# apple/ml-neuman

Hardware: AMD Instinct MI355X
Metric: rays_per_sec (800x800 frame, 128 samples/ray coarse + 128 importance, NeuMan background NeRF) (higher is better)
Workload: dtype coarse (sampling) pass: split-fp16 hi+lo MFMA x3, f32 accumulate; fine (shading) pass: per-row-scaled int16 as two int8 limbs on the i8 MFMA x3, exact int32 accumulate, encodings on split bf16

## Files before the change

ml-neuman_amd/csrc/mlp_host.hip:

```cpp
#include <stdarg.h>
#include <stdio.h>
#include <stdlib.h>
#include <string.h>

#include <vector>

#include "common.h"
#include "mlp_layout.h"
#include "mlp_launch.h"

namespace nm {

static thread_local char g_err[512] = "";

void set_error(const char* fmt, ...) {
    va_list ap;
    va_start(ap, fmt);
    vsnprintf(g_err, sizeof(g_err), fmt, ap);
    va_end(ap);
}
int check_hip(hipError_t e, const char* what) {
    if (e == hipSuccess) return NM_OK;
    set_error("%s: %s", what, hipGetErrorString(e));
    return NM_ERR_HIP;
// ... 302 lines not shown
                                int v = (int)lrintf(w / q[n]);
                                if (v > kFixedMax) v = kFixedMax;
                                if (v < -kFixedMax) v = -kFixedMax;
                                const int l = ((v + 128) & 255) - 128;
                                const int h = (v - l) >> 8;
                                hi[(g * 32 + r) * 16 + e] = (int8_t)h;
                                lo[(g * 32 + r) * 16 + e] = (int8_t)l;
                            }
                    }
                }
        }
        for (int n = 0; n < nrows; ++n) b[n] /= u[n];
        for (int nb = 0; nb < sh.nblk; ++nb)
            for (int t = 0; t < sh.bfsteps; ++t) {
                uint16_t* hi = reinterpret_cast<uint16_t*>(img + frag_off8(st, nb, sh.i8steps + t));
                uint16_t* lo = hi + 64 * 8;
                const int cc0 = st == 9 ? 32 : 0;
                for (int lane = 0; lane < 64; ++lane)
                    for (int j = 0; j < 8; ++j) {
                        const int n = 32 * nb + (lane & 31);
                        const float wv = stage_weight(d, P, st, n, cc0 + 2 * t + (lane >> 5), j) / u[n];
                        const uint16_t h = f32_to_bf16(wv);
                        hi[lane * 8 + j] = h;
                        lo[lane * 8 + j] = f32_to_bf16(wv - bf16_to_f32(h));
                    }
            }
    }
}

static void pack_stream8s(const uint8_t* img8, uint8_t* out, bool plain = false) {
    memset(out, 0, (size_t)(kWeightBytes8 + kWeightPadBytes));
    uint8_t* dst = out;
    auto put = [&](int st, int nb, int t0, int n) {
        for (int t = 0; t < n; ++t, dst += kStepBytes) memcpy(dst, img8 + frag_off8(st, nb, t0 + t), (size_t)kStepBytes);
    };
    for (int nb = 0; nb < 8; ++nb) put(0, nb, 0, 4);
    for (int st = 1; st <= 7; ++st) {
        for (int nb = 0; nb < 8; ++nb) put(st, nb, 0, 8);
        if (st == 5)
            for (int nb = 0; nb < 8; ++nb) put(5, nb, 8, 4);
    }
    put(8, 8, 0, 8);
    if (plain) {
        for (int nb = 0; nb < 2; ++nb) { put(0, nb, 0, 4); dst += 4 * kStepBytes; }
        if (dst - out != kPlainStreamBytes8) abort();
        return;
    }
    for (int nb = 0; nb < 8; ++nb) put(8, nb, 0, 8);
    for (int nb = 0; nb < 4; ++nb) put(9, nb, 0, 10);
    put(10, 0, 0, 4);
    if (dst - out != kWeightBytes8) abort();
}

constexpr int kSigmaSteps = 8 * 4 + 6 * 8 * 16 + 8 * 20 + 16;
static void sigma_stream_table(std::vector<int>& tab, int ndir) {
    tab.clear();
    std::vector<int> direct;
    auto put = [&](int st, int b, int t0, int n) {
        for (int t = 0; t < n; ++t)
            for (int k = 0; k < 4; ++k) {
                const int off = (int)frag_off(st, b + (k >> 1), t0 + t) + 1024 * (k & 1);
                (k < 4 - ndir ? tab : direct).push_back(off);
            }
    };
    for (int st = 0; st <= 7; ++st) {
        const StageShape sh = stage_shape(st);
        for (int b = 0; b < 8; b += 2) {
            if (sh.pe_steps) put(st, b, 0, sh.pe_steps);
            for (int t0 = sh.pe_steps; t0 < sh.steps; t0 += 8) put(st, b, t0, 8);
        }
    }
    for (int t = 0; t < 16; ++t) { tab.push_back((int)frag_off(8, 8, t)); tab.push_back((int)frag_off(8, 8, t) + 1024); }
    tab.insert(tab.end(), direct.begin(), direct.end());
    if ((int)tab.size() != 2 * kSigmaSteps) abort();
}
__global__ void sigma_stream_kernel(const uint4* __restrict__ image, const int* __restrict__ tab, int npieces, uint4* __restrict__ out) {
    const int i = blockIdx.x * blockDim.x + threadIdx.x;
    if (i >= npieces * 64) return;
    out[i] = image[tab[i >> 6] / 16 + (i & 63)];
}

static void pack_stream8(const uint8_t* img8, uint8_t* out) {
    memset(out, 0, (size_t)kWeightBytes8w);
    for (int q = 0; q < 4; ++q) {
        uint8_t* dst = out + wstream_off(q);
        auto put = [&](int st, int nb, int t0, int n) {
            for (int t = 0; t < n; ++t, dst += kStepBytes) memcpy(dst, img8 + frag_off8(st, nb, t0 + t), (size_t)kStepBytes);
        };
        put(0, 2 * q, 0, 4); put(0, 2 * q + 1, 0, 4);
        for (int st = 1; st <= 8; ++st) {
            put(st, 2 * q, 0, 8); put(st, 2 * q + 1, 0, 8);
            if (st == 5) { put(5, 2 * q, 8, 4); put(5, 2 * q + 1, 8, 4); }
        }
        if (q < 2) put(8, 8, 0, 8);
        put(9, q, 0, 8); put(9, q, 8, 2);
        dst += 2 * kStepBytes;
        if (q < 2) put(10, 0, 0, 4);
        dst += kW8Pad * kStepBytes;
        if (dst != out + wstream_off(q) + (int64_t)wstream_steps(q) * kStepBytes) abort();
    }
}

}

struct nm_mlp_s {
    nm_mlp_desc desc;
// ... 39 lines not shown
int nm_mlp_pack_f16(const nm_mlp_desc* desc, const float* const* host_params, void* host_out) {
    if (int e = nm::validate_desc(desc)) return e;
    NM_REQUIRE(host_params && host_out, "nm_mlp_pack_f16: null pointer");
    for (int i = 0; i < (desc->plain_head ? 18 : 24); ++i) NM_REQUIRE(host_params[i], "nm_mlp_pack_f16: host_params[%d] is null", i);
    nm::pack_image(desc, host_params, static_cast<uint8_t*>(host_out), true);
    return NM_OK;
}

int64_t nm_mlp_pack_i8_bytes(const nm_mlp_desc* desc) {
    if (nm::validate_desc(desc) != NM_OK) return -1;
    return nm::image8_bytes();
}

int nm_mlp_pack_i8(const nm_mlp_desc* desc, const float* const* host_params, void* host_out) {
    if (int e = nm::validate_desc(desc)) return e;
    NM_REQUIRE(host_params && host_out, "nm_mlp_pack_i8: null pointer");
    for (int i = 0; i < (desc->plain_head ? 18 : 24); ++i) NM_REQUIRE(host_params[i], "nm_mlp_pack_i8: host_params[%d] is null", i);
    nm::pack_image8(desc, host_params, static_cast<uint8_t*>(host_out));
    return NM_OK;
}

int64_t nm_mlp_pack_i8s_bytes(const nm_mlp_desc* desc) {
    if (nm::validate_desc(desc) != NM_OK) return -1;
    return nm::kWeightBytes8 + nm::kWeightPadBytes;
}

int nm_mlp_pack_i8s(const nm_mlp_desc* desc, const float* const* host_params, void* host_out) {
    if (int e = nm::validate_desc(desc)) return e;
    NM_REQUIRE(host_params && host_out, "nm_mlp_pack_i8s: null pointer");
    for (int i = 0; i < (desc->plain_head ? 18 : 24); ++i) NM_REQUIRE(host_params[i], "nm_mlp_pack_i8s: host_params[%d] is null", i);
    std::vector<uint8_t> img8((size_t)nm::image8_bytes());
    nm::pack_image8(desc, host_params, img8.data());
    nm::pack_stream8s(img8.data(), static_cast<uint8_t*>(host_out), desc->plain_head != 0);
    return NM_OK;
}

int nm_mlp_create(const nm_mlp_desc* desc, const float* const* host_params, const float* host_pos_tab,
                  const float* host_dir_tab, nm_mlp_t* out) {
    if (int e = nm::validate_desc(desc)) return e;
    NM_REQUIRE(host_params && host_pos_tab && host_dir_tab && out, "nm_mlp_create: null pointer");
    const int plain = desc->plain_head;
    for (int i = 0; i < (plain ? 18 : 24); ++i) NM_REQUIRE(host_params[i], "nm_mlp_create: host_params[%d] is null", i);
    const int64_t bytes = nm_mlp_pack_bytes(desc);
    std::vector<uint8_t> img((size_t)bytes);
    nm::pack_image(desc, host_params, img.data());
    std::vector<uint8_t> img16((size_t)bytes);
    nm::pack_image(desc, host_params, img16.data(), true);
    std::vector<uint8_t> img8((size_t)nm::image8_bytes());
    std::vector<uint8_t> str8((size_t)nm::kWeightBytes8w);
    std::vector<uint8_t> str8s((size_t)(nm::kWeightBytes8 + nm::kWeightPadBytes));
    nm::pack_image8(desc, host_params, img8.data());
    nm::pack_stream8(img8.data(), str8.data());
    nm::pack_stream8s(img8.data(), str8s.data(), plain != 0);

    const int kpe = 3 + 6 * desc->pos_n_freqs, kdpe = 3 + 6 * desc->dir_n_freqs;
    const int K[12] = {kpe, 256, 256, 256, 256, kpe + 256, 256, 256, plain ? 0 : 256 + kdpe, plain ? 0 : 256, 256, plain ? 0 : 128};
    const int N[12] = {256, 256, 256, 256, 256, 256, 256, 256, plain ? 0 : 128, plain ? 0 : 256, plain ? 4 : 1, plain ? 0 : 3};
    const int src[12] = {0, 2, 4, 6, 8, 10, 12, 14, 16, 18, plain ? (int)nm::P_OUT_W : 20, 22};
    nm_mlp_s* m = new nm_mlp_s();
    m->desc = *desc;
    int woff = 0;
    for (int l = 0; l < 12; ++l) { m->ref_off[l] = woff; woff += K[l] * N[l]; }
    int boff = woff;
    for (int l = 0; l < 12; ++l) { m->ref_boff[l] = boff; boff += N[l]; }
    std::vector<float> ref((size_t)boff);
    for (int l = 0; l < 12; ++l) {
        if (!K[l]) continue;
        const float* W = host_params[src[l]];
        for (int k = 0; k < K[l]; ++k)
            for (int n = 0; n < N[l]; ++n) ref[m->ref_off[l] + (size_t)k * N[l] + n] = W[(size_t)n * K[l] + k];
        memcpy(&ref[m->ref_boff[l]], host_params[src[l] + 1], (size_t)N[l] * 4);
    }
    float tab[192];
    memset(tab, 0, sizeof(tab));
    const int npos = desc->pe_kind == NM_PE_POSENC ? desc->pos_n_freqs : 9 * desc->pos_n_freqs;
    const int ndir = desc->pe_kind == NM_PE_POSENC ? desc->dir_n_freqs : 9 * desc->dir_n_freqs;
    memcpy(tab, host_pos_tab, (size_t)npos * 4);
    memcpy(tab + 96, host_dir_tab, (size_t)ndir * 4);
    auto octaves = [&](const float* t, int nfreq) {
        const int per = desc->pe_kind == NM_PE_POSENC ? 1 : 9;
        for (int b = 0; b + 1 < nfreq; ++b)
            for (int k = 0; k < per; ++k)
                if (t[(b + 1) * per + k] != 2.f * t[b * per + k]) return 0;
        return 1;
    };
    m->pos_octaves = octaves(tab, desc->pos_n_freqs);
    m->dir_octaves = octaves(tab + 96, desc->dir_n_freqs);

    m->d_image = nullptr; m->d_image16 = nullptr; m->d_consts8 = nullptr; m->d_stream8 = nullptr; m->d_image8 = nullptr; m->d_stream16t = nullptr; m->d_sigma_tab = nullptr; m->d_bwd_image = nullptr; m->d_petab = nullptr; m->d_ref = nullptr; m->d_wscale16 = nullptr;
    int rc = nm::check_hip(hipMalloc(&m->d_image, (size_t)bytes), "nm_mlp_create: hipMalloc(image)");
    const size_t consts_off = (size_t)(nm::kWeightBytes8 + nm::kWeightPadBytes), consts_bytes = img8.size() - consts_off;
    if (!rc) rc = nm::check_hip(hipMalloc(&m->d_consts8, consts_bytes), "nm_mlp_create: hipMalloc(consts8)");
    if (!rc) rc = nm::check_hip(hipMemcpy(m->d_consts8, img8.data() + consts_off, consts_bytes, hipMemcpyHostToDevice), "nm_mlp_create: upload consts8");
    if (!rc) rc = nm::check_hip(hipMalloc(&m->d_stream8, str8.size()), "nm_mlp_create: hipMalloc(stream8)");
    if (!rc) rc = nm::check_hip(hipMemcpy(m->d_stream8, str8.data(), str8.size(), hipMemcpyHostToDevice), "nm_mlp_create: upload stream8");
    if (!rc) rc = nm::check_hip(hipMalloc(&m->d_image8, consts_off), "nm_mlp_create: hipMalloc(image8)");
    if (!rc) rc = nm::check_hip(hipMemcpy(m->d_image8, str8s.data(), consts_off, hipMemcpyHostToDevice), "nm_mlp_create: upload image8");
    if (!rc) rc = nm::check_hip(hipMalloc(&m->d_petab, sizeof(tab)), "nm_mlp_create: hipMalloc(petab)");
    if (!rc) rc = nm::check_hip(hipMalloc(&m->d_ref, ref.size() * 4), "nm_mlp_create: hipMalloc(ref)");
    if (!rc) rc = nm::check_hip(hipMemcpy(m->d_image, img.data(), (size_t)bytes, hipMemcpyHostToDevice), "nm_mlp_create: upload image");
    if (!rc) rc = nm::check_hip(hipMalloc(&m->d_image16, (size_t)bytes), "nm_mlp_create: hipMalloc(image16)");
    if (!rc) rc = nm::check_hip(hipMemcpy(m->d_image16, img16.data(), (size_t)bytes, hipMemcpyHostToDevice), "nm_mlp_create: upload image16");
    if (!rc) rc = nm::check_hip(hipMemcpy(m->d_petab, tab, sizeof(tab), hipMemcpyHostToDevice), "nm_mlp_create: upload petab");
    if (!rc) rc = nm::check_hip(hipMemcpy(m->d_ref, ref.data(), ref.size() * 4, hipMemcpyHostToDevice), "nm_mlp_create: upload ref");
    if (!rc && !plain) {
        std::vector<int> stab;
// ... 42 lines not shown
}

int nm_mlp_destroy(nm_mlp_t m) {
    if (!m) return NM_OK;
    if (m->d_image) (void)hipFree(m->d_image);
    if (m->d_image16) (void)hipFree(m->d_image16);
    if (m->d_consts8) (void)hipFree(m->d_consts8);
    if (m->d_stream8) (void)hipFree(m->d_stream8);
    if (m->d_image8) (void)hipFree(m->d_image8);
    if (m->d_stream16t) (void)hipFree(m->d_stream16t);
    if (m->d_sigma_tab) (void)hipFree(m->d_sigma_tab);
    if (m->d_bwd_image) (void)hipFree(m->d_bwd_image);
    if (m->d_petab) (void)hipFree(m->d_petab);
    if (m->d_ref) (void)hipFree(m->d_ref);
    if (m->d_wscale16) (void)hipFree(m->d_wscale16);
    delete m;
    return NM_OK;
}

static int mlp_dispatch(nm_mlp_t m, const float* pts, const float* dirs, const float* origin, const float* direction,
                        const float* z, int64_t n, int S, int in_mode, int precision, int stop_stage, float sigma_scale,
                        float* out, float* dbg, nm_stream_t stream, void* prof = nullptr, int sigma_only = 0,
                        const nm::MlpChunk* chunk = nullptr) {
    NM_REQUIRE(m, "nm_mlp_forward: null handle");
    NM_REQUIRE(n >= 0, "nm_mlp_forward: negative n");
    NM_REQUIRE(precision == NM_PREC_FP32 || precision == NM_PREC_BF16X3 || precision == NM_PREC_BF16 || precision == NM_PREC_I8X3 ||
                   precision == NM_PREC_FP16X3,
               "nm_mlp_forward: bad precision %d", precision);
    if (n == 0) return NM_OK;
    NM_REQUIRE(!(chunk && precision == NM_PREC_FP32), "nm_mlp_forward_ray_chunk: the exact-f32 validation kernel has no chunked form");
    NM_REQUIRE(!(m->desc.plain_head && precision == NM_PREC_I8X3 && (stop_stage != -2 || dbg || prof || sigma_only)),
               "nm_mlp_forward: the plain-head (use_viewdirs=False) net's i8x3 form is the whole-network launch only (no stage-by-stage / density-only form)");
    NM_REQUIRE(!(m->desc.plain_head && stop_stage > 7), "nm_mlp_forward_debug: the plain-head net has stages -1..7 only");
    if (precision == NM_PREC_FP32) {
        nm::RefLaunch L;
        L.plain_head = m->desc.plain_head;
        L.wt = m->d_ref; L.bias = m->d_ref; L.petab = m->d_petab;
        for (int i = 0; i < 12; ++i) { L.off[i] = m->ref_off[i]; L.boff[i] = m->ref_boff[i]; }
        L.pe_kind = m->desc.pe_kind; L.pos_nfreq = m->desc.pos_n_freqs; L.dir_nfreq = m->desc.dir_n_freqs;
        return nm::launch_mlp_ref(L, pts, dirs, origin, direction, z, n, S, in_mode, stop_stage, sigma_scale, out, dbg,
                                  nm::as_stream(stream));
    }
    nm::MlpLaunch L;
    L.wpack = m->d_image;
    L.bias = reinterpret_cast<const float*>(m->d_image + nm::kWeightBytes + nm::kWeightPadBytes);
    L.wpack16 = m->d_image16;
    L.bias16 = reinterpret_cast<const float*>(m->d_image16 + nm::kWeightBytes + nm::kWeightPadBytes);
    L.petab = m->d_petab;
    L.pe_kind = m->desc.pe_kind; L.pos_nfreq = m->desc.pos_n_freqs; L.dir_nfreq = m->desc.dir_n_freqs;
    L.pos_octaves = m->pos_octaves; L.dir_octaves = m->dir_octaves;
    L.plain_head = m->desc.plain_head;
    L.wstream8 = m->d_stream8;
    L.consts8 = m->d_consts8;
    static const bool i8_as = [] { const char* e = getenv("NEUMAN_I8_KERNEL"); return !e || !strcmp(e, "as"); }();
    const char* sk = getenv("NEUMAN_SIGMA_KERNEL");
    const bool sigma_t = !(sk && !strcmp(sk, "w")) && m->d_stream16t;
    if (sigma_t && precision == NM_PREC_FP16X3 && sigma_only == 1 && stop_stage == -2 && !dbg && !prof && !m->desc.plain_head)
        return nm::launch_sigma_f16t(L, m->d_stream16t, m->sigma_ndir, pts, dirs, origin, direction, z, n, S, in_mode, sigma_scale, out, nm::as_stream(stream), chunk, nullptr, -1);
    if ((i8_as || m->desc.plain_head) && precision == NM_PREC_I8X3 && stop_stage == -2 && !dbg && !prof && !sigma_only)
        return nm::launch_mlp_i8s(L, m->d_image8, pts, dirs, origin, direction, z, n, S, in_mode, sigma_scale, out, nm::as_stream(stream), chunk);
    return nm::launch_mlp_mfma(L, pts, dirs, origin, direction, z, n, S, in_mode, precision, stop_stage, sigma_scale, out, dbg,
                               prof, nm::as_stream(stream), sigma_only, chunk);
}

int nm_mlp_forward(nm_mlp_t mlp, const float* pts, const float* dirs, int64_t n, int precision, float sigma_scale,
                   float* out, nm_stream_t stream) {
    NM_REQUIRE(n == 0 || (pts && dirs && out), "nm_mlp_forward: null pointer");
    NM_REQUIRE((reinterpret_cast<uintptr_t>(out) & 15) == 0, "nm_mlp_forward: out must be 16-byte aligned");
    return mlp_dispatch(mlp, pts, dirs, nullptr, nullptr, nullptr, n, 1, 0, precision, -2, sigma_scale, out, nullptr, stream);
}

int nm_mlp_forward_save(nm_mlp_t m, const float* pts, const float* dirs, int64_t n, float* save_h, float* save_hv, float* out,
                        nm_stream_t stream) {
    return nm_mlp_forward_save_bits(m, pts, dirs, n, save_h, save_hv, nullptr, out, stream);
}

static int forward_save_impl(nm_mlp_t m, const float* pts, const float* dirs, int64_t n, float* save_h, float* save_hv, uint32_t* save_bits,
                             void* save_h16, float* out, nm_stream_t stream, void* save_feat16 = nullptr, uint32_t* save_hvbits = nullptr,
                             void* save_x0h = nullptr, void* save_d0h = nullptr) {
    NM_REQUIRE(m, "nm_mlp_forward_save: null handle");
    NM_REQUIRE(n >= 0, "nm_mlp_forward_save: negative n");
    if (n == 0) return NM_OK;
    const bool plain = m->desc.plain_head != 0;
    NM_REQUIRE(!plain || (save_h16 && !save_h && !save_feat16 && !save_hvbits && !save_d0h), "nm_mlp_forward_save: the plain-head net keeps save_h16 / save_bits / save_x0h only");
    NM_REQUIRE(pts && (dirs || plain) && (plain || ((save_h || (save_h16 && save_feat16)) && save_hv)) && out, "nm_mlp_forward_save: null pointer");
    NM_REQUIRE(((reinterpret_cast<uintptr_t>(out) | reinterpret_cast<uintptr_t>(save_h) | reinterpret_cast<uintptr_t>(save_hv) | reinterpret_cast<uintptr_t>(save_h16) |
                 reinterpret_cast<uintptr_t>(save_feat16)) & 15) == 0, "nm_mlp_forward_save: outputs must be 16-byte aligned");
    nm::MlpLaunch L;
    L.wpack = m->d_image;
    L.bias = reinterpret_cast<const float*>(m->d_image + nm::kWeightBytes + nm::kWeightPadBytes);
    L.wpack16 = m->d_image16;
    L.bias16 = reinterpret_cast<const float*>(m->d_image16 + nm::kWeightBytes + nm::kWeightPadBytes);
    L.petab = m->d_petab;
    L.pe_kind = m->desc.pe_kind; L.pos_nfreq = m->desc.pos_n_freqs; L.dir_nfreq = m->desc.dir_n_freqs;
    L.pos_octaves = m->pos_octaves; L.dir_octaves = m->dir_octaves;
    L.plain_head = plain ? 1 : 0;
    L.wstream8 = m->d_stream8;
    L.consts8 = m->d_consts8;
    L.save_h = save_h; L.save_hv = save_hv; L.save_bits = save_bits; L.save_h16 = save_h16; L.save_feat16 = save_feat16; L.save_hvbits = save_hvbits; L.save_x0h = save_x0h; L.save_d0h = save_d0h;
    return nm::launch_mlp_mfma(L, pts, dirs ? dirs : pts, nullptr, nullptr, nullptr, n, 1, 0, NM_PREC_FP16X3, -2, 1.f, out, nullptr, nullptr,
                               nm::as_stream(stream), 0, nullptr);
}

int nm_mlp_forward_save_bits(nm_mlp_t m, const float* pts, const float* dirs, int64_t n, float* save_h, float* save_hv, uint32_t* save_bits,
                             float* out, nm_stream_t stream) {
    return forward_save_impl(m, pts, dirs, n, save_h, save_hv, save_bits, nullptr, out, stream);
}
// ... 215 lines not shown
```

ml-neuman_amd/csrc/mlp_i8s.hip:

```cpp
#include "mlp_i8as.h"
#include <stdio.h>
#include <stdlib.h>
#include <vector>

namespace {

constexpr int kWaves = 8;
constexpr int kTile = kWaves * kRows;
constexpr int kPWaveU4 = nm::kPeChunks * 2 * kRows;
constexpr int kPeU4 = kWaves * kPWaveU4;
constexpr int kStepU4 = nm::kStepBytes / 16;
constexpr int kSlotU4 = 12 * kStepU4;
constexpr int kSlots = 3;
constexpr int kBiasU4 = (nm::kBiasFloats + 16 + 3) / 4;
constexpr int kTileBlocks = 82;
__host__ __device__ constexpr int block_steps(int i) {
    i = i >= kTileBlocks ? i - kTileBlocks : i;
    return i < 8 ? 4 : i < 77 ? 8 : i < 81 ? 10 : 4;
}
__host__ __device__ constexpr int block_pieces(int nsteps) { return (2 * nsteps + kWaves - 1) / kWaves; }

#ifdef NM_AS_PROF
struct Prof {
    unsigned long long t, acc[8];
};
#define PROF_DECL Prof P; P.t = __builtin_amdgcn_s_memtime(); for (int i_ = 0; i_ < 8; ++i_) P.acc[i_] = 0;
#define PROF_TICK(b) { const unsigned long long n_ = __builtin_amdgcn_s_memtime(); P.acc[b] += n_ - P.t; P.t = n_; }
#define PROF_ARG , Prof& P
#define PROF_PASS , P
#else
#define PROF_DECL
#define PROF_TICK(b)
#define PROF_ARG
#define PROF_PASS
#endif
struct Ring {
    const char* src;
    const uint4* rd;
    unsigned lds0;
    int off;
    int slot;
    int refill, np, nsteps2;
};
__device__ __forceinline__ void ring_piece(const Ring& R, int off, int slot, int j) {
    glds16(R.src + off + j * (kWaves * 1024), __builtin_amdgcn_readfirstlane(R.lds0 + slot * (kSlotU4 * 16) + j * (kWaves * 1024)));
}
__device__ __forceinline__ void ring_advance(Ring& R, int nsteps) {
    R.off += nsteps * nm::kStepBytes;
    if (R.off == (int)nm::kWeightBytes8) R.off = 0;
}
__device__ __forceinline__ const uint4* ring_enter(Ring& R, int i PROF_ARG) {
    PROF_TICK(4)
    const int np1 = block_pieces(block_steps(i + 1));
    if (np1 == 1) asm volatile("s_waitcnt vmcnt(1)" ::: "memory");
    else if (np1 == 2) asm volatile("s_waitcnt vmcnt(2)" ::: "memory");
    else asm volatile("s_waitcnt vmcnt(3)" ::: "memory");
    __builtin_amdgcn_s_barrier();
    PROF_TICK(0)
    const uint4* cur = R.rd + R.slot * kSlotU4;
    R.refill = R.slot == 0 ? kSlots - 1 : R.slot - 1;
    R.slot = R.slot == kSlots - 1 ? 0 : R.slot + 1;
    R.np = block_pieces(block_steps(i + 2));
    R.nsteps2 = block_steps(i + 2);
    return cur;
}
__device__ __forceinline__ void ring_copy(Ring& R, int j) {
    if (j < R.np) ring_piece(R, R.off, R.refill, j);
    if (j == R.np - 1) ring_advance(R, R.nsteps2);
}
struct W8 {
    uint4 h, l;
};

template <int NSTEPS, bool PEND, bool RELU = true>
__device__ __forceinline__ void k_i8_impl(i32x16& t, const X8& X, const uint4* ws, Ring& R, f32x16& fp, const i32x16& tp, lds_cfloat* bias_blk,
                                          float sx256, float& m) {
    i32x16 ah, ac;
#pragma unroll
    for (int r = 0; r < 16; ++r) { ah[r] = 0; ac[r] = 0; }
    W8 w[2];
    w[0].h = ws[0]; w[0].l = ws[64];
    w[1].h = ws[kStepU4]; w[1].l = ws[kStepU4 + 64];
#pragma unroll
    for (int s = 0; s < NSTEPS; ++s) {
        const uint4 wh = w[s & 1].h, wl = w[s & 1].l;
        ac = __builtin_amdgcn_mfma_i32_32x32x32_i8(as_i32x4(wh), as_i32x4(X.l[s]), ac, 0, 0, 0);
        ah = __builtin_amdgcn_mfma_i32_32x32x32_i8(as_i32x4(wh), as_i32x4(X.h[s]), ah, 0, 0, 0);
        ac = __builtin_amdgcn_mfma_i32_32x32x32_i8(as_i32x4(wl), as_i32x4(X.h[s]), ac, 0, 0, 0);
        if (s + 2 < NSTEPS) { w[s & 1].h = ws[(s + 2) * kStepU4]; w[s & 1].l = ws[(s + 2) * kStepU4 + 64]; }
        if (s == 0 || s == 2 || s == 4) ring_copy(R, s >> 1);
        if (PEND) {
            const int r = 2 * s;
            const float b0 = bias_blk[8 * (r >> 2) + (r & 3)], b1 = bias_blk[8 * (r >> 2) + (r & 3) + 1];
            const float f0 = fmaf((float)tp[r], sx256, b0), f1 = fmaf((float)tp[r + 1], sx256, b1);
            fp[r] = f0;
            fp[r + 1] = f1;
            m = RELU ? fmaxf(m, fmaxf(f0, f1)) : fmaxf(m, fmaxf(fabsf(f0), fabsf(f1)));
            __builtin_amdgcn_sched_barrier(0);
        }
    }
#pragma unroll
    for (int r = 0; r < 16; ++r) t[r] = (ah[r] << 8) + ac[r];
}
template <int NSTEPS>
__device__ __forceinline__ void k_i8(i32x16& t, const X8& X, const uint4* ws, Ring& R) {
    f32x16 nf;
    float nm_ = 0.f;
    k_i8_impl<NSTEPS, false>(t, X, ws, R, nf, t, nullptr, 0.f, nm_);
}
template <int NSTEPS, bool COPY = false>
__device__ __forceinline__ void k_bf(f32x16& f, const uint4* pw, int g, int s, const uint4* ws, Ring* R = nullptr, int j0 = 0) {
#pragma unroll
    for (int t = 0; t < NSTEPS; ++t) {
        if (COPY && (t == 1 || t == 3)) ring_copy(*R, j0 + (t >> 1));
        const uint4 wh = ws[t * kStepU4], wl = ws[t * kStepU4 + 64];
        const uint4 xh = pw[(2 * t + g) * (2 * kRows) + s], xl = pw[(2 * t + g) * (2 * kRows) + kRows + s];
        f = __builtin_amdgcn_mfma_f32_32x32x16_bf16(as_bf16x8(wh), as_bf16x8(xl), f, 0, 0, 0);
        f = __builtin_amdgcn_mfma_f32_32x32x16_bf16(as_bf16x8(wl), as_bf16x8(xh), f, 0, 0, 0);
        f = __builtin_amdgcn_mfma_f32_32x32x16_bf16(as_bf16x8(wh), as_bf16x8(xh), f, 0, 0, 0);
    }
}
template <bool PLAIN>
__global__ __launch_bounds__(kWaves * 64, 2) void nerf_mlp_i8s_kernel(const Args8s A) {
    __shared__ uint4 lds[kPeU4 + kSlots * kSlotU4 + kBiasU4];
    const MlpArgs a = resolve_args(A.a);
    const int tid = threadIdx.x, lane = tid & 63;
    const int w = __builtin_amdgcn_readfirstlane(tid >> 6);
    const int g = lane >> 5, s = lane & 31;
    uint4* pw = lds + w * kPWaveU4;
    Ring R;
    R.src = reinterpret_cast<const char*>(A.image8) + lane * 16 + w * 1024;
    R.rd = lds + kPeU4 + lane;
    R.lds0 = (unsigned)(uintptr_t)(lds + kPeU4) + w * 1024;
    R.off = 0;
    R.slot = 0;
    {
        float* lb = reinterpret_cast<float*>(lds + kPeU4 + kSlots * kSlotU4);
        for (int i = tid; i < nm::kBiasFloats + 16; i += kWaves * 64) lb[i] = A.consts8[nm::kBiasFloats + i];
    }
    __syncthreads();
    ring_piece(R, 0, 0, 0);
    ring_piece(R, block_steps(0) * nm::kStepBytes, 1, 0);
    R.off = (block_steps(0) + block_steps(1)) * nm::kStepBytes;
    const float u_sigma = A.consts8[nm::stage_b_off(8) + 256];
    const float u_r = A.consts8[nm::stage_b_off(10)], u_g = A.consts8[nm::stage_b_off(10) + 1], u_b = A.consts8[nm::stage_b_off(10) + 2];
    const float* kappa = reinterpret_cast<const float*>(lds + kPeU4 + kSlots * kSlotU4) + nm::kBiasFloats;
    unsigned bias_lds = (unsigned)(uintptr_t)(lds + kPeU4 + kSlots * kSlotU4) + 16 * g;
    asm volatile("" : "+v"(bias_lds));
    lds_cfloat* bias = (lds_cfloat*)(uintptr_t)bias_lds;
    const int64_t ntiles = (a.n + kTile - 1) / kTile;
    for (int i = lane; i < kPWaveU4; i += 64) pw[i] = make_uint4(0, 0, 0, 0);
    PROF_DECL

#pragma unroll 1
    for (int64_t tile = blockIdx.x; tile < ntiles; tile += gridDim.x) {
        const int64_t row0 = tile * kTile + w * kRows;
        PROF_TICK(7)
        fill_pe_wave(pw, false, a, row0, lane);
        PROF_TICK(6)
        X8 X;
        float sx;
        {
            f32x16 f[8];
            float m = 0.f;
#pragma unroll
            for (int b = 0; b < 8; ++b) {
                const uint4* ws = ring_enter(R, b PROF_PASS);
                bias16(f[b], bias + nm::stage_b_off(0) + 32 * b);
                k_bf<4, true>(f[b], pw, g, s, ws, &R);
                PROF_TICK(2)
                m = max16<true>(m, f[b]);
            }
            PROF_TICK(4)
            const float M = row_max(m), inv = inv_of(M);
#pragma unroll
            for (int b = 0; b < 8; ++b) quant16<true>(f[b], inv, X.h[b], X.l[b]);
            sx = scale_of(M);
            PROF_TICK(5)
        }
#pragma unroll 1
        for (int st = 1; st <= 7; ++st) {
            const float sxin = sx * (256.f * kappa[st]);
            const int i0 = 8 * st + (st > 5 ? 4 : 0);
            f32x16 f[8];
            float m = 0.f;
            i32x16 tp;
#pragma unroll
            for (int b = 0; b < 8; ++b) {
                const uint4* ws = ring_enter(R, i0 + b PROF_PASS);
                if (b == 0) {
                    k_i8<8>(tp, X, ws, R);
                } else {
                    i32x16 t;
                    k_i8_impl<8, true>(t, X, ws, R, f[b - 1], tp, bias + 256 * st + 32 * (b - 1), sxin, m);
                    tp = t;
                }
                PROF_TICK(2)
            }
            dequant16(f[7], tp, sxin, bias + 256 * st + 32 * 7);
            if (st == 5) {
#pragma unroll
                for (int u = 0; u < 4; ++u) {
                    const uint4* ws = ring_enter(R, 48 + u PROF_PASS);
                    k_bf<4, true>(f[2 * u], pw, g, s, ws, &R, 0);
                    k_bf<4, true>(f[2 * u + 1], pw, g, s, ws + 4 * kStepU4, &R, 2);
                    PROF_TICK(2)
                }
                m = 0.f;
#pragma unroll
                for (int b = 0; b < 7; ++b) m = max16<true>(m, f[b]);
            }
            m = max16<true>(m, f[7]);
            PROF_TICK(4)
            const float M = row_max(m), inv = inv_of(M);
#pragma unroll
            for (int b = 0; b < 8; ++b) quant16<true>(f[b], inv, X.h[b], X.l[b]);
            sx = scale_of(M);
            PROF_TICK(5)
            if (st == 5 && !(PLAIN && a.sigma_only == 2)) {
                PROF_TICK(7)
                fill_pe_wave(pw, true, a, row0, lane);
                PROF_TICK(6)
            }
        }
        if (PLAIN && a.sigma_only == 2) {
            i32x16 t;
            f32x16 fo;
            k_i8<8>(t, X, ring_enter(R, 68 PROF_PASS), R);
            PROF_TICK(2)
            dequant16(fo, t, sx * (256.f * kappa[8]), bias + nm::stage_b_off(8) + 256);
            const float* up = A.consts8 + nm::stage_b_off(8) + 256;
            const int64_t i = row0 + s;
            if (g == 0 && i < a.n)
                reinterpret_cast<float4*>(a.out)[sample_record(a, i)] = make_float4(fo[0] * up[0], fo[1] * up[1], fo[2] * up[2], fo[3] * up[3] * a.sigma_scale);
            R.off = (block_steps(0) + block_steps(1)) * nm::kStepBytes;
            continue;
        }
        float sigma;
        {
            const float sxin = sx * (256.f * kappa[8]);
            {
                i32x16 t;
                f32x16 fa;
                k_i8<8>(t, X, ring_enter(R, 68 PROF_PASS), R);
                PROF_TICK(2)
                dequant16(fa, t, sxin, bias + nm::stage_b_off(8) + 256);
                sigma = fa[0] * u_sigma;
            }
            f32x16 f[8];
            float m = 0.f;
#pragma unroll
            for (int b = 0; b < 8; ++b) {
                i32x16 t;
                k_i8<8>(t, X, ring_enter(R, 69 + b PROF_PASS), R);
                PROF_TICK(2)
                dequant16(f[b], t, sxin, bias + nm::stage_b_off(8) + 32 * b);
                m = max16<false>(m, f[b]);
            }
            PROF_TICK(4)
            const float M = row_max(m), inv = inv_of(M);
#pragma unroll
            for (int b = 0; b < 8; ++b) quant16<false>(f[b], inv, X.h[b], X.l[b]);
            sx = scale_of(M);
            PROF_TICK(5)
        }
        {
            const float sxin = sx * (256.f * kappa[9]);
            f32x16 f[4];
            float m = 0.f;
#pragma unroll
            for (int b = 0; b < 4; ++b) {
                i32x16 t;
                const uint4* ws = ring_enter(R, 77 + b PROF_PASS);
                k_i8<8>(t, X, ws, R);
                PROF_TICK(2)
                dequant16(f[b], t, sxin, bias + nm::stage_b_off(9) + 32 * b);
                k_bf<2>(f[b], pw, g, s, ws + 8 * kStepU4);
                m = max16<true>(m, f[b]);
            }
            PROF_TICK(4)
            const float M = row_max(m), inv = inv_of(M);
#pragma unroll
            for (int b = 0; b < 4; ++b) quant16<true>(f[b], inv, X.h[b], X.l[b]);
            sx = scale_of(M);
            PROF_TICK(5)
        }
        {
            i32x16 t;
            f32x16 fr;
            k_i8<4>(t, X, ring_enter(R, 81 PROF_PASS), R);
            PROF_TICK(2)
            dequant16(fr, t, sx * (256.f * kappa[10]), bias + nm::stage_b_off(10));
            const int64_t i = row0 + s;
            if (g == 0 && i < a.n)
                reinterpret_cast<float4*>(a.out)[sample_record(a, i)] =
                    make_float4(fr[0] * u_r, fr[1] * u_g, fr[2] * u_b,
                                sigma * a.sigma_scale);
        }
    }
#ifdef NM_AS_PROF
    PROF_TICK(7)
    if (lane == 0 && a.prof)
        for (int i = 0; i < 8; ++i) a.prof[((size_t)blockIdx.x * kWaves + w) * 8 + i] = P.acc[i];
#endif
    asm volatile("s_waitcnt vmcnt(0)" ::: "memory");
}

}

namespace nm {

int launch_mlp_i8s(const MlpLaunch& L, const void* image8, const float* pts, const float* dirs, const float* origin, const float* direction,
                   const float* z, int64_t n, int S, int in_mode, float sigma_scale, float* out, hipStream_t stream, const MlpChunk* chunk) {
    Args8s A;
    MlpArgs& a = A.a;
    a.ray_idx = chunk ? chunk->ray_idx : nullptr;
    a.n_rays_dev = chunk ? chunk->n_rays_dev : nullptr;
    a.s0 = chunk ? chunk->s0 : 0;
    a.S_total = chunk ? chunk->S_total : S;
    a.wpack = nullptr; a.bias = nullptr;
    a.petab = L.petab;
    a.pts = pts; a.dirs = dirs; a.origin = origin; a.direction = direction; a.z = z;
    a.out = out; a.dbg = nullptr; a.prof = nullptr; a.n = n; a.S = S; a.in_mode = in_mode; a.stop_stage = -2; a.sigma_scale = sigma_scale;
    a.sigma_only = L.plain_head ? 2 : 0;
    a.save_h = nullptr; a.save_hv = nullptr; a.save_bits = nullptr; a.save_h16 = nullptr; a.save_feat16 = nullptr; a.save_hvbits = nullptr; a.save_x0h = nullptr; a.save_d0h = nullptr;
    a.pos = PeSpec{L.pe_kind, L.pos_nfreq, L.pos_octaves};
    a.dir = PeSpec{L.pe_kind, L.dir_nfreq, L.dir_octaves};
    A.consts8 = L.consts8;
    A.image8 = reinterpret_cast<const uint4*>(image8);
    const int64_t ntiles = (n + kTile - 1) / kTile;
    int dev = 0, cus = 256;
    if (hipGetDevice(&dev) == hipSuccess) {
        int v = 0;
        if (hipDeviceGetAttribute(&v, hipDeviceAttributeMultiprocessorCount, dev) == hipSuccess && v > 0) cus = v;
    }
    const int grid = (int)(ntiles < cus ? ntiles : cus);
    if (getenv("NEUMAN_I8S_DEBUG")) {
        int nb = -1;
        hipError_t e = hipOccupancyMaxActiveBlocksPerMultiprocessor(&nb, nerf_mlp_i8s_kernel<false>, kWaves * 64, 0);
        fprintf(stderr, "nerf_mlp_i8s_kernel: occupancy %d blocks/CU (%s), grid %d, cus %d\n", nb, hipGetErrorString(e), grid, cus);
    }
#ifdef NM_AS_PROF
    static unsigned long long* d_prof = nullptr;
    const size_t nprof = (size_t)grid * kWaves * 8;
    if (!d_prof) (void)hipMalloc(&d_prof, (size_t)1024 * kWaves * 8 * 8);
    (void)hipMemsetAsync(d_prof, 0, nprof * 8, stream);
    a.prof = d_prof;
#endif
    if (L.plain_head) hipLaunchKernelGGL(nerf_mlp_i8s_kernel<true>, dim3(grid), dim3(kWaves * 64), 0, stream, A);
    else hipLaunchKernelGGL(nerf_mlp_i8s_kernel<false>, dim3(grid), dim3(kWaves * 64), 0, stream, A);
#ifdef NM_AS_PROF
    if (n > 1000000) {
        std::vector<unsigned long long> h(nprof);
        (void)hipStreamSynchronize(stream);
        (void)hipMemcpy(h.data(), d_prof, nprof * 8, hipMemcpyDeviceToHost);
        static const char* names[8] = {"top barrier", "copy issue", "k-loop", "-", "epilogue", "requantise", "encodings", "rest"};
        double acc[8] = {0}, tot = 0;
        for (size_t i = 0; i < nprof; ++i) acc[i & 7] += (double)h[i];
        for (int i = 0; i < 8; ++i) tot += acc[i];
        fprintf(stderr, "mean cycles per wave %.0f:", tot / (grid * (double)kWaves));
        for (int i = 0; i < 8; ++i) fprintf(stderr, "  %s %.1f%%", names[i], 100.0 * acc[i] / tot);
        fprintf(stderr, "\n");
    }
#endif
    return check_launch("nerf_mlp_i8s_kernel");
}

}
```

ml-neuman_amd/csrc/mlp_launch.h:

```cpp
#pragma once
#include "common.h"

namespace nm {

enum { P_OUT_W = 16, P_OUT_B = 17 };
enum { P_PTS_W = 0, P_VIEWS_W = 16, P_VIEWS_B = 17, P_FEAT_W = 18, P_FEAT_B = 19, P_ALPHA_W = 20, P_ALPHA_B = 21, P_RGB_W = 22, P_RGB_B = 23 };
struct DevParams {
    const float* p[24];
};

struct MlpLaunch {
    const void* wpack; const float* bias; const float* petab;
    int pe_kind, pos_nfreq, dir_nfreq;
    int pos_octaves, dir_octaves;
    int plain_head;
    const void* wpack16; const float* bias16;
    const void* wstream8; const float* consts8;
    float* save_h = nullptr;
    float* save_hv = nullptr;
    unsigned* save_bits = nullptr;
    void* save_h16 = nullptr;
    void* save_feat16 = nullptr;
    unsigned* save_hvbits = nullptr;
    void* save_x0h = nullptr; void* save_d0h = nullptr;
};
struct RefLaunch {
    const float* wt; const float* bias; int off[12]; int boff[12]; const float* petab;
    int pe_kind, pos_nfreq, dir_nfreq;
    int plain_head;
};

struct MlpChunk {
    const int* ray_idx; const int* n_rays_dev; int s0, S_total;
};

int launch_mlp_mfma(const MlpLaunch& L, const float* pts, const float* dirs, const float* origin, const float* direction,
                    const float* z, int64_t n, int S, int in_mode, int precision, int stop_stage, float sigma_scale, float* out,
                    float* dbg, void* prof, hipStream_t stream, int sigma_only = 0, const MlpChunk* chunk = nullptr);
int launch_mlp_i8s(const MlpLaunch& L, const void* image8, const float* pts, const float* dirs, const float* origin, const float* direction,
                   const float* z, int64_t n, int S, int in_mode, float sigma_scale, float* out, hipStream_t stream, const MlpChunk* chunk);
int sigma_f16t_ndir();
int launch_sigma_f16t(const MlpLaunch& L, const void* stream16t, int stream_ndir, const float* pts, const float* dirs, const float* origin, const float* direction,
                      const float* z, int64_t n, int S, int in_mode, float sigma_scale, float* out, hipStream_t stream, const MlpChunk* chunk,
                      float* dbg, int dbg_stage);
int64_t mlp_bwd_image_bytes();
struct Bwd16 {
    void* dz16; void* dfeat16; const float* amax; float* dz32[8];
    const unsigned* hvbits = nullptr; void* dhv16 = nullptr; float* dhv32 = nullptr; int kdir = 0;
    int plain = 0;
};
int launch_mlp_bwd(const DevParams& P, int kpe, uint8_t* image, const float* dz_top, const float* d_feat, const float* d_raw, const float* acts,
                   const unsigned* relu_bits, int64_t n, float* dz_out, float* colsum, float* gb, hipStream_t stream, const Bwd16* h = nullptr);
int launch_mlp_ref(const RefLaunch& L, const float* pts, const float* dirs, const float* origin, const float* direction,
                   const float* z, int64_t n, int S, int in_mode, int stop_stage, float sigma_scale, float* out, float* dbg,
                   hipStream_t stream);

}
```

Baseline: 1.462 million.

## Use 16x16x64 i8 MFMA in fine-pass kernel with repacked weight stream

Adds a Q16 variant of the int8 fine-pass kernel that replaces each 32x32x32 i8 MFMA with two 16x16x64 i8 MFMAs on sub-blocks of the accumulator. On the host, the int8 weight stream is repacked into the matching lane layout. Activations are reshuffled with permlane16_swap after each requantisation, and results are swapped back after accumulation. The new variant is on by default and can be turned off with NEUMAN_I8_KERNEL=as32. It aims for higher MFMA throughput but adds extra lane-swap and accumulator shuffling work.

```diff
diff --git a/ml-neuman_amd/csrc/mlp_host.hip b/ml-neuman_amd/csrc/mlp_host.hip
--- a/ml-neuman_amd/csrc/mlp_host.hip
+++ b/ml-neuman_amd/csrc/mlp_host.hip
@@ -378,6 +378,37 @@
     if (dst - out != kWeightBytes8) abort();
 }
 
+static void pack_stream8q(const uint8_t* s8s, uint8_t* out, bool plain = false) {
+    memcpy(out, s8s, (size_t)(kWeightBytes8 + kWeightPadBytes));
+    int64_t off = 0;
+    auto i8 = [&](int nsteps) {
+        for (int q = 0; 2 * q < nsteps; ++q, off += 2 * kStepBytes)
+            for (int h = 0; h < 2; ++h)
+                for (int L = 0; L < 2; ++L)
+                    for (int lane = 0; lane < 64; ++lane) {
+                        const int c = lane >> 4, m = lane & 15;
+                        const int row = 16 * h + 8 * ((m >> 2) & 1) + 4 * (m >> 3) + (m & 3);
+                        memcpy(out + off + h * kStepBytes + L * 1024 + lane * 16,
+                               s8s + off + (c & 1) * kStepBytes + L * 1024 + (32 * (c >> 1) + row) * 16, 16);
+                    }
+    };
+    auto skip = [&](int nsteps) { off += (int64_t)nsteps * kStepBytes; };
+    skip(8 * 4);
+    for (int st = 1; st <= 7; ++st) {
+        for (int nb = 0; nb < 8; ++nb) i8(8);
+        if (st == 5) skip(8 * 4);
+    }
+    i8(8);
+    if (plain) {
+        if (off + 2 * 8 * kStepBytes != kPlainStreamBytes8) abort();
+        return;
+    }
+    for (int nb = 0; nb < 8; ++nb) i8(8);
+    for (int nb = 0; nb < 4; ++nb) { i8(8); skip(2); }
+    i8(4);
+    if (off != kWeightBytes8) abort();
+}
+
 constexpr int kSigmaSteps = 8 * 4 + 6 * 8 * 16 + 8 * 20 + 16;
 static void sigma_stream_table(std::vector<int>& tab, int ndir) {
     tab.clear();
@@ -523,6 +554,11 @@
     nm::pack_image8(desc, host_params, img8.data());
     nm::pack_stream8(img8.data(), str8.data());
     nm::pack_stream8s(img8.data(), str8s.data(), plain != 0);
+    if (nm::i8s_q16()) {
+        std::vector<uint8_t> str8q(str8s.size());
+        nm::pack_stream8q(str8s.data(), str8q.data(), plain != 0);
+        str8s.swap(str8q);
+    }
 
     const int kpe = 3 + 6 * desc->pos_n_freqs, kdpe = 3 + 6 * desc->dir_n_freqs;
     const int K[12] = {kpe, 256, 256, 256, 256, kpe + 256, 256, 256, plain ? 0 : 256 + kdpe, plain ? 0 : 256, 256, plain ? 0 : 128};
@@ -671,7 +707,7 @@
     L.plain_head = m->desc.plain_head;
     L.wstream8 = m->d_stream8;
     L.consts8 = m->d_consts8;
-    static const bool i8_as = [] { const char* e = getenv("NEUMAN_I8_KERNEL"); return !e || !strcmp(e, "as"); }();
+    static const bool i8_as = [] { const char* e = getenv("NEUMAN_I8_KERNEL"); return !e || !strcmp(e, "as") || !strcmp(e, "as32"); }();
     const char* sk = getenv("NEUMAN_SIGMA_KERNEL");
     const bool sigma_t = !(sk && !strcmp(sk, "w")) && m->d_stream16t;
     if (sigma_t && precision == NM_PREC_FP16X3 && sigma_only == 1 && stop_stage == -2 && !dbg && !prof && !m->desc.plain_head)
diff --git a/ml-neuman_amd/csrc/mlp_i8s.hip b/ml-neuman_amd/csrc/mlp_i8s.hip
--- a/ml-neuman_amd/csrc/mlp_i8s.hip
+++ b/ml-neuman_amd/csrc/mlp_i8s.hip
@@ -1,6 +1,7 @@
 #include "mlp_i8as.h"
 #include <stdio.h>
 #include <stdlib.h>
+#include <string.h>
 #include <vector>
 
 namespace {
@@ -72,7 +73,31 @@
     uint4 h, l;
 };
 
-template <int NSTEPS, bool PEND, bool RELU = true>
+__device__ __forceinline__ void swap16(int& a, int& b) {
+    const auto v = __builtin_amdgcn_permlane16_swap((unsigned)a, (unsigned)b, false, false);
+    a = (int)v[0];
+    b = (int)v[1];
+}
+__device__ __forceinline__ void swap16(unsigned& a, unsigned& b) {
+    const auto v = __builtin_amdgcn_permlane16_swap(a, b, false, false);
+    a = v[0];
+    b = v[1];
+}
+template <int NSTEPS>
+__device__ __forceinline__ void to_b16(X8& X) {
+    auto pair = [](uint4& a, uint4& b) {
+        unsigned a0 = a.x, a1 = a.y, a2 = a.z, a3 = a.w, b0 = b.x, b1 = b.y, b2 = b.z, b3 = b.w;
+        swap16(a0, b0); swap16(a1, b1); swap16(a2, b2); swap16(a3, b3);
+        a = make_uint4(a0, a1, a2, a3);
+        b = make_uint4(b0, b1, b2, b3);
+    };
+#pragma unroll
+    for (int q = 0; 2 * q < NSTEPS; ++q) {
+        pair(X.h[2 * q], X.h[2 * q + 1]);
+        pair(X.l[2 * q], X.l[2 * q + 1]);
+    }
+}
+template <int NSTEPS, bool PEND, bool RELU = true, bool Q16 = false>
 __device__ __forceinline__ void k_i8_impl(i32x16& t, const X8& X, const uint4* ws, Ring& R, f32x16& fp, const i32x16& tp, lds_cfloat* bias_blk,
                                           float sx256, float& m) {
     i32x16 ah, ac;
@@ -84,9 +109,23 @@
 #pragma unroll
     for (int s = 0; s < NSTEPS; ++s) {
         const uint4 wh = w[s & 1].h, wl = w[s & 1].l;
-        ac = __builtin_amdgcn_mfma_i32_32x32x32_i8(as_i32x4(wh), as_i32x4(X.l[s]), ac, 0, 0, 0);
-        ah = __builtin_amdgcn_mfma_i32_32x32x32_i8(as_i32x4(wh), as_i32x4(X.h[s]), ah, 0, 0, 0);
-        ac = __builtin_amdgcn_mfma_i32_32x32x32_i8(as_i32x4(wl), as_i32x4(X.h[s]), ac, 0, 0, 0);
+        if constexpr (Q16) {
+            const int h = s & 1, q2 = s & ~1, o0 = 8 * h, o1 = 8 * h + 4;
+            i32x4 c0 = {ac[o0], ac[o0 + 1], ac[o0 + 2], ac[o0 + 3]}, c1 = {ac[o1], ac[o1 + 1], ac[o1 + 2], ac[o1 + 3]};
+            i32x4 d0 = {ah[o0], ah[o0 + 1], ah[o0 + 2], ah[o0 + 3]}, d1 = {ah[o1], ah[o1 + 1], ah[o1 + 2], ah[o1 + 3]};
+            c0 = __builtin_amdgcn_mfma_i32_16x16x64_i8(as_i32x4(wh), as_i32x4(X.l[q2]), c0, 0, 0, 0);
+            c1 = __builtin_amdgcn_mfma_i32_16x16x64_i8(as_i32x4(wh), as_i32x4(X.l[q2 + 1]), c1, 0, 0, 0);
+            d0 = __builtin_amdgcn_mfma_i32_16x16x64_i8(as_i32x4(wh), as_i32x4(X.h[q2]), d0, 0, 0, 0);
+            d1 = __builtin_amdgcn_mfma_i32_16x16x64_i8(as_i32x4(wh), as_i32x4(X.h[q2 + 1]), d1, 0, 0, 0);
+            c0 = __builtin_amdgcn_mfma_i32_16x16x64_i8(as_i32x4(wl), as_i32x4(X.h[q2]), c0, 0, 0, 0);
+            c1 = __builtin_amdgcn_mfma_i32_16x16x64_i8(as_i32x4(wl), as_i32x4(X.h[q2 + 1]), c1, 0, 0, 0);
+#pragma unroll
+            for (int i = 0; i < 4; ++i) { ac[o0 + i] = c0[i]; ac[o1 + i] = c1[i]; ah[o0 + i] = d0[i]; ah[o1 + i] = d1[i]; }
+        } else {
+            ac = __builtin_amdgcn_mfma_i32_32x32x32_i8(as_i32x4(wh), as_i32x4(X.l[s]), ac, 0, 0, 0);
+            ah = __builtin_amdgcn_mfma_i32_32x32x32_i8(as_i32x4(wh), as_i32x4(X.h[s]), ah, 0, 0, 0);
+            ac = __builtin_amdgcn_mfma_i32_32x32x32_i8(as_i32x4(wl), as_i32x4(X.h[s]), ac, 0, 0, 0);
+        }
         if (s + 2 < NSTEPS) { w[s & 1].h = ws[(s + 2) * kStepU4]; w[s & 1].l = ws[(s + 2) * kStepU4 + 64]; }
         if (s == 0 || s == 2 || s == 4) ring_copy(R, s >> 1);
         if (PEND) {
@@ -101,12 +140,25 @@
     }
 #pragma unroll
     for (int r = 0; r < 16; ++r) t[r] = (ah[r] << 8) + ac[r];
-}
-template <int NSTEPS>
+    if constexpr (Q16) {
+        i32x16 v;
+#pragma unroll
+        for (int h = 0; h < 2; ++h)
+#pragma unroll
+            for (int i = 0; i < 4; ++i) {
+                int a0 = t[8 * h + i], a1 = t[8 * h + 4 + i];
+                swap16(a0, a1);
+                v[8 * h + i] = a0;
+                v[8 * h + 4 + i] = a1;
+            }
+        t = v;
+    }
+}
+template <int NSTEPS, bool Q16>
 __device__ __forceinline__ void k_i8(i32x16& t, const X8& X, const uint4* ws, Ring& R) {
     f32x16 nf;
     float nm_ = 0.f;
-    k_i8_impl<NSTEPS, false>(t, X, ws, R, nf, t, nullptr, 0.f, nm_);
+    k_i8_impl<NSTEPS, false, true, Q16>(t, X, ws, R, nf, t, nullptr, 0.f, nm_);
 }
 template <int NSTEPS, bool COPY = false>
 __device__ __forceinline__ void k_bf(f32x16& f, const uint4* pw, int g, int s, const uint4* ws, Ring* R = nullptr, int j0 = 0) {
@@ -120,7 +172,7 @@
         f = __builtin_amdgcn_mfma_f32_32x32x16_bf16(as_bf16x8(wh), as_bf16x8(xh), f, 0, 0, 0);
     }
 }
-template <bool PLAIN>
+template <bool PLAIN, bool Q16>
 __global__ __launch_bounds__(kWaves * 64, 2) void nerf_mlp_i8s_kernel(const Args8s A) {
     __shared__ uint4 lds[kPeU4 + kSlots * kSlotU4 + kBiasU4];
     const MlpArgs a = resolve_args(A.a);
@@ -175,6 +227,7 @@
             const float M = row_max(m), inv = inv_of(M);
 #pragma unroll
             for (int b = 0; b < 8; ++b) quant16<true>(f[b], inv, X.h[b], X.l[b]);
+            if constexpr (Q16) to_b16<8>(X);
             sx = scale_of(M);
             PROF_TICK(5)
         }
@@ -189,10 +242,10 @@
             for (int b = 0; b < 8; ++b) {
                 const uint4* ws = ring_enter(R, i0 + b PROF_PASS);
                 if (b == 0) {
-                    k_i8<8>(tp, X, ws, R);
+                    k_i8<8, Q16>(tp, X, ws, R);
                 } else {
                     i32x16 t;
-                    k_i8_impl<8, true>(t, X, ws, R, f[b - 1], tp, bias + 256 * st + 32 * (b - 1), sxin, m);
+                    k_i8_impl<8, true, true, Q16>(t, X, ws, R, f[b - 1], tp, bias + 256 * st + 32 * (b - 1), sxin, m);
                     tp = t;
                 }
                 PROF_TICK(2)
@@ -215,6 +268,7 @@
             const float M = row_max(m), inv = inv_of(M);
 #pragma unroll
             for (int b = 0; b < 8; ++b) quant16<true>(f[b], inv, X.h[b], X.l[b]);
+            if constexpr (Q16) to_b16<8>(X);
             sx = scale_of(M);
             PROF_TICK(5)
             if (st == 5 && !(PLAIN && a.sigma_only == 2)) {
@@ -226,7 +280,7 @@
         if (PLAIN && a.sigma_only == 2) {
             i32x16 t;
             f32x16 fo;
-            k_i8<8>(t, X, ring_enter(R, 68 PROF_PASS), R);
+            k_i8<8, Q16>(t, X, ring_enter(R, 68 PROF_PASS), R);
             PROF_TICK(2)
             dequant16(fo, t, sx * (256.f * kappa[8]), bias + nm::stage_b_off(8) + 256);
             const float* up = A.consts8 + nm::stage_b_off(8) + 256;
@@ -242,7 +296,7 @@
             {
                 i32x16 t;
                 f32x16 fa;
-                k_i8<8>(t, X, ring_enter(R, 68 PROF_PASS), R);
+                k_i8<8, Q16>(t, X, ring_enter(R, 68 PROF_PASS), R);
                 PROF_TICK(2)
                 dequant16(fa, t, sxin, bias + nm::stage_b_off(8) + 256);
                 sigma = fa[0] * u_sigma;
@@ -252,7 +306,7 @@
 #pragma unroll
             for (int b = 0; b < 8; ++b) {
                 i32x16 t;
-                k_i8<8>(t, X, ring_enter(R, 69 + b PROF_PASS), R);
+                k_i8<8, Q16>(t, X, ring_enter(R, 69 + b PROF_PASS), R);
                 PROF_TICK(2)
                 dequant16(f[b], t, sxin, bias + nm::stage_b_off(8) + 32 * b);
                 m = max16<false>(m, f[b]);
@@ -261,6 +315,7 @@
             const float M = row_max(m), inv = inv_of(M);
 #pragma unroll
             for (int b = 0; b < 8; ++b) quant16<false>(f[b], inv, X.h[b], X.l[b]);
+            if constexpr (Q16) to_b16<8>(X);
             sx = scale_of(M);
             PROF_TICK(5)
         }
@@ -272,7 +327,7 @@
             for (int b = 0; b < 4; ++b) {
                 i32x16 t;
                 const uint4* ws = ring_enter(R, 77 + b PROF_PASS);
-                k_i8<8>(t, X, ws, R);
+                k_i8<8, Q16>(t, X, ws, R);
                 PROF_TICK(2)
                 dequant16(f[b], t, sxin, bias + nm::stage_b_off(9) + 32 * b);
                 k_bf<2>(f[b], pw, g, s, ws + 8 * kStepU4);
@@ -282,13 +337,14 @@
             const float M = row_max(m), inv = inv_of(M);
 #pragma unroll
             for (int b = 0; b < 4; ++b) quant16<true>(f[b], inv, X.h[b], X.l[b]);
+            if constexpr (Q16) to_b16<4>(X);
             sx = scale_of(M);
             PROF_TICK(5)
         }
         {
             i32x16 t;
             f32x16 fr;
-            k_i8<4>(t, X, ring_enter(R, 81 PROF_PASS), R);
+            k_i8<4, Q16>(t, X, ring_enter(R, 81 PROF_PASS), R);
             PROF_TICK(2)
             dequant16(fr, t, sx * (256.f * kappa[10]), bias + nm::stage_b_off(10));
             const int64_t i = row0 + s;
@@ -309,6 +365,11 @@
 }
 
 namespace nm {
+
+bool i8s_q16() {
+    static const bool q16 = [] { const char* e = getenv("NEUMAN_I8_KERNEL"); return !(e && !strcmp(e, "as32")); }();
+    return q16;
+}
 
 int launch_mlp_i8s(const MlpLaunch& L, const void* image8, const float* pts, const float* dirs, const float* origin, const float* direction,
                    const float* z, int64_t n, int S, int in_mode, float sigma_scale, float* out, hipStream_t stream, const MlpChunk* chunk) {
@@ -337,7 +398,7 @@
     const int grid = (int)(ntiles < cus ? ntiles : cus);
     if (getenv("NEUMAN_I8S_DEBUG")) {
         int nb = -1;
-        hipError_t e = hipOccupancyMaxActiveBlocksPerMultiprocessor(&nb, nerf_mlp_i8s_kernel<false>, kWaves * 64, 0);
+        hipError_t e = hipOccupancyMaxActiveBlocksPerMultiprocessor(&nb, nerf_mlp_i8s_kernel<false, true>, kWaves * 64, 0);
         fprintf(stderr, "nerf_mlp_i8s_kernel: occupancy %d blocks/CU (%s), grid %d, cus %d\n", nb, hipGetErrorString(e), grid, cus);
     }
 #ifdef NM_AS_PROF
@@ -347,8 +408,11 @@
     (void)hipMemsetAsync(d_prof, 0, nprof * 8, stream);
     a.prof = d_prof;
 #endif
-    if (L.plain_head) hipLaunchKernelGGL(nerf_mlp_i8s_kernel<true>, dim3(grid), dim3(kWaves * 64), 0, stream, A);
-    else hipLaunchKernelGGL(nerf_mlp_i8s_kernel<false>, dim3(grid), dim3(kWaves * 64), 0, stream, A);
+    const bool q16 = i8s_q16();
+    if (L.plain_head && q16) hipLaunchKernelGGL(HIP_KERNEL_NAME(nerf_mlp_i8s_kernel<true, true>), dim3(grid), dim3(kWaves * 64), 0, stream, A);
+    else if (L.plain_head) hipLaunchKernelGGL(HIP_KERNEL_NAME(nerf_mlp_i8s_kernel<true, false>), dim3(grid), dim3(kWaves * 64), 0, stream, A);
+    else if (q16) hipLaunchKernelGGL(HIP_KERNEL_NAME(nerf_mlp_i8s_kernel<false, true>), dim3(grid), dim3(kWaves * 64), 0, stream, A);
+    else hipLaunchKernelGGL(HIP_KERNEL_NAME(nerf_mlp_i8s_kernel<false, false>), dim3(grid), dim3(kWaves * 64), 0, stream, A);
 #ifdef NM_AS_PROF
     if (n > 1000000) {
         std::vector<unsigned long long> h(nprof);
diff --git a/ml-neuman_amd/csrc/mlp_launch.h b/ml-neuman_amd/csrc/mlp_launch.h
--- a/ml-neuman_amd/csrc/mlp_launch.h
+++ b/ml-neuman_amd/csrc/mlp_launch.h
@@ -37,6 +37,7 @@
 int launch_mlp_mfma(const MlpLaunch& L, const float* pts, const float* dirs, const float* origin, const float* direction,
                     const float* z, int64_t n, int S, int in_mode, int precision, int stop_stage, float sigma_scale, float* out,
                     float* dbg, void* prof, hipStream_t stream, int sigma_only = 0, const MlpChunk* chunk = nullptr);
+bool i8s_q16();
 int launch_mlp_i8s(const MlpLaunch& L, const void* image8, const float* pts, const float* dirs, const float* origin, const float* direction,
                    const float* z, int64_t n, int S, int in_mode, float sigma_scale, float* out, hipStream_t stream, const MlpChunk* chunk);
 int sigma_f16t_ndir();
```

Result: no change. 1.468 million (median of 6 runs) (+0.4%).
